# aoschu/esn-ofdm-mimo

Measured on AMD Instinct MI355X. Metric: OFDM symbols/s through the ESN detector (4x8 TDL-B, N=128, N_res=512; train+predict+detect), higher is better.
Workload: dtype f16 operands / f32 accumulate

## Files before the change

### esn_ofdm_mimo_amd/csrc/esn_api.hip

```cpp
#include <stdarg.h>
#include <stdio.h>
#include <stdlib.h>
#include <math.h>
#include <string.h>
#include "esn_common.h"

namespace esn {
int launch_recur_f64(const RecurParams& p, hipStream_t stream);
size_t recur_f64_lds_bytes(int FB, int n_res, int n_in, int n_out);
bool f64_mfma_geometry(int n_res, int n_in, int n_out, bool harvest, Geometry* g);
int launch_recur_f64_mfma(const RecurParams& p, hipStream_t stream);
#ifdef ESN_WITH_RS
bool rs_path_applies(int precision, const RecurParams& p);
int launch_recur_rs(int precision, const RecurParams& p, size_t wo_rs_off, hipStream_t stream);
#endif
bool big_path_applies(int precision, const RecurParams& p);
int big_slots(const RecurParams& p);
size_t big_workspace_bytes(int n_slots, int Mp, int Kp);
int launch_recur_big(int precision, const RecurParams& p, size_t wo_big_off, void* workspace, hipStream_t stream,
                     bool io32 = false);
bool big_harvest_applies(int precision, const RecurParams& p);
size_t big_harvest_workspace_bytes(int n_groups, int Kp);
int launch_harvest_big(int precision, const RecurParams& p, void* workspace, hipStream_t stream);
bool cluster_applies(int precision, const RecurParams& p);
size_t cluster_workspace_bytes(int n_res, int n_in, int n_out, bool harvest);
int launch_recur_cluster(const RecurParams& p, void* workspace, hipStream_t stream);
bool mfma_geometry(int precision, int n_res, int n_in, int n_out, bool harvest, Geometry* g);
int launch_recur_mfma(int precision, const RecurParams& p, hipStream_t stream, bool io32 = false);
bool harvest_cluster_applies(int precision, const RecurParams& p);
size_t harvest_cluster_workspace_bytes(int n_pilots, int C, int n_wsets);
int launch_harvest_cluster(int precision, const RecurParams& p, int C, void* workspace, hipStream_t stream);
int launch_recur_skew16(int precision, const RecurParams& p, hipStream_t stream, bool io32 = false);
size_t packed_w_bytes(int precision, int n_res, int n_in, int n_out, const Geometry& g);
size_t packed_wout_bytes(int precision, int n_res, int n_in, int n_out, const Geometry& g);
size_t wout_big_offset(int precision, int n_out, const Geometry& g);
size_t f64_w_offset(int n_res, int n_in, int n_out);
size_t f64_wout_offset(int n_res, int n_in, int n_out);
int launch_pack_weights(int precision, const esn_shape_t* sh, const Geometry& g, const double* W,
                        const double* Win, const double* Wfb, void* packed, hipStream_t stream);
int launch_pack_readout(int precision, const esn_shape_t* sh, const Geometry& g, int n_groups,
                        const double* Wout, void* packed, hipStream_t stream);
size_t solve_work_doubles(int rows, int cols, int n_out);
int launch_readout_solve(const double* E, const double* D, int n_groups, int T, int transient,
                         int cols, int n_out, const double* t_scale, const double* t_shift,
                         double* W_out, int* status, void* workspace, hipStream_t stream);
int launch_readout_chol(const double* E, const float* E32, const double* D, int n_groups, int T, int transient,
                        int cols, int n_out, const double* t_scale, const double* t_shift,
                        double* W_out, int* status, hipStream_t stream);
size_t chol_big_work_doubles(int n);
int launch_readout_chol_big(const double* E, const float* E32, const double* D, int n_groups, int T, int transient,
                            int cols, int n_out, const double* t_scale, const double* t_shift,
                            double* W_out, int* status, void* workspace, hipStream_t stream);
int launch_gen_taps(const TapParams& tp, hipStream_t stream);
int launch_gen_frames(const FrameGenParams& fp, hipStream_t stream, bool c64 = false);
int launch_channel_estimate(const ChanEstParams& cp, hipStream_t stream);
int launch_mmse_detect(const MmseParams& mp, hipStream_t stream);
int launch_taps_to_freq(const TapsFreqParams& tp, hipStream_t stream);
int launch_ldpc_encode(const LdpcEncodeParams& ep, hipStream_t stream);
int launch_qam_llr(const LlrParams& lp, hipStream_t stream);
int launch_ldpc_decode(const LdpcDecodeParams& dp, hipStream_t stream);
int launch_detect_count(const DetectParams& dp, hipStream_t stream, bool io32 = false);
}

using namespace esn;

static thread_local char g_err[512] = "";

namespace esn {
static bool parse3(const char* v, int (&out)[3]) {
    int a, b, c;
    if (v && sscanf(v, "%d,%d,%d", &a, &b, &c) == 3 && a > 0 && b > 0 && c > 0) { out[0] = a; out[1] = b; out[2] = c; return true; }
    out[0] = out[1] = out[2] = 0;
    return false;
}
Knobs& knobs() {
    static Knobs k = [] {
        Knobs x;
        const char* v = getenv("ESN_SKEW");
        x.skew = (v && v[0] == '0') ? 0 : 1;
        parse3(getenv("ESN_MFMA_GEOM"), x.geom16);
        parse3(getenv("ESN_MFMA_GEOM_F32"), x.geom32);
        v = getenv("ESN_CHOL_SKIP");
        x.chol_skip = v ? atoi(v) : 0;
        v = getenv("ESN_F64_MFMA");
        x.f64_mfma = (v && v[0] == '0') ? 0 : 1;
        v = getenv("ESN_RS");
        x.rs = (v && v[0] == '1') ? 1 : 0;
        v = getenv("ESN_BIG_GEMM");
        x.big_gemm = (v && v[0] == '0') ? 0 : 1;
        v = getenv("ESN_CLUSTER");
        x.cluster = (v && v[0] == '0') ? 0 : 1;
        x.gen_ko = 0;
        v = getenv("ESN_HARVEST_GEMM");
        x.harvest_gemm = (v && v[0] == '1') ? 1 : 0;
        v = getenv("ESN_BIG_NT");
        x.big_nt = (v && v[0] == '4') ? 4 : 2;
        v = getenv("ESN_HCLUSTER");
        x.hcluster = (v && (v[0] == '0' || v[0] == '4' || v[0] == '8')) ? v[0] - '0' : 1;
        v = getenv("ESN_S16");
        x.s16 = (v && v[0] == '0') ? 0 : 1;
        v = getenv("ESN_BIG_PIPE");
        x.big_pipe = (v && v[0] == '0') ? 0 : 1;
        return x;
    }();
    return k;
}
}

static int fail(int code, const char* fmt, ...) {
    va_list ap;
    va_start(ap, fmt);
    vsnprintf(g_err, sizeof(g_err), fmt, ap);
    va_end(ap);
    return code;
}

namespace esn {
int api_fail(int code, const char* fmt, ...) {
    va_list ap;
    va_start(ap, fmt);
    vsnprintf(g_err, sizeof(g_err), fmt, ap);
    va_end(ap);
    return code;
}
}

static int hip_fail(int e, const char* what) {
    if (e == 0) return 0;
    if (e > 0) return fail(-1000 - e, "%s: HIP error %d (%s)", what, e, hipGetErrorString((hipError_t)e));
    return fail(-2, "%s: no kernel instance for this shape", what);
}

static bool check_shape(const esn_shape_t* s) {
    return s && s->n_res > 0 && s->n_in > 0 && s->n_out > 0 && s->n_wsets > 0;
}

static bool geometry_for(int precision, const esn_shape_t* s, Geometry* g, bool harvest = false) {
    memset(g, 0, sizeof(*g));
    if (precision == ESN_F64) {
        int fb = 8;
        while (fb > 1 && recur_f64_lds_bytes(fb, s->n_res, s->n_in, s->n_out) > 150 * 1024) fb >>= 1;
        if (recur_f64_lds_bytes(fb, s->n_res, s->n_in, s->n_out) > 160 * 1024) return false;
        Geometry gp, gh;
        memset(&gp, 0, sizeof(gp)); memset(&gh, 0, sizeof(gh));
        if (f64_mfma_geometry(s->n_res, s->n_in, s->n_out, false, &gp) &&
            f64_mfma_geometry(s->n_res, s->n_in, s->n_out, true, &gh))
            *g = harvest ? gh : gp;
        g->Bt = fb;
        return true;
    }
    if (precision < ESN_F64 || precision > ESN_BF16) return false;
    return mfma_geometry(precision, s->n_res, s->n_in, s->n_out, harvest, g);
}

#ifdef ESN_STAMPS
static unsigned long long* g_stamp_buf = nullptr;
extern "C" void esn_debug_set_stamp_buffer(void* dev) { g_stamp_buf = (unsigned long long*)dev; }
#define ESN_SET_STAMPS(p) (p).stamps = g_stamp_buf
#else
#define ESN_SET_STAMPS(p) (p).stamps = nullptr
#endif

extern "C" {

const char* esn_last_error(void) { return g_err; }

int esn_abi_version(void) { return 10; }

int esn_debug_set(const char* key, const char* value) {
    if (!key) return fail(-1, "esn_debug_set: null key");
    Knobs& k = knobs();
    if (!strcmp(key, "skew")) { k.skew = (value && value[0] == '0') ? 0 : 1; return 0; }
    if (!strcmp(key, "mfma_geom")) { parse3(value, k.geom16); return 0; }
    if (!strcmp(key, "mfma_geom_f32")) { parse3(value, k.geom32); return 0; }
    if (!strcmp(key, "chol_skip")) { k.chol_skip = value ? atoi(value) : 0; return 0; }
    if (!strcmp(key, "f64_mfma")) { k.f64_mfma = (value && value[0] == '0') ? 0 : 1; return 0; }
    if (!strcmp(key, "rs")) {
#ifdef ESN_WITH_RS
        k.rs = (value && value[0] == '1') ? 1 : 0; return 0;
#else
        if (value && value[0] == '1') return fail(-3, "esn_debug_set: the register-state kernel is not in this build (ESN_WITH_RS=1)");
        return 0;
#endif
    }
    if (!strcmp(key, "big_gemm")) { k.big_gemm = (value && value[0] == '0') ? 0 : 1; return 0; }
    if (!strcmp(key, "cluster")) { k.cluster = (value && value[0] == '0') ? 0 : 1; return 0; }
    if (!strcmp(key, "gen_ko")) { k.gen_ko = value ? atoi(value) : 0; return 0; }
    if (!strcmp(key, "harvest_gemm")) { k.harvest_gemm = (value && value[0] == '1') ? 1 : 0; return 0; }
    if (!strcmp(key, "big_nt")) { k.big_nt = (value && value[0] == '4') ? 4 : 2; return 0; }
    if (!strcmp(key, "hcluster")) {
        k.hcluster = (value && (value[0] == '0' || value[0] == '4' || value[0] == '8')) ? value[0] - '0' : 1;
        return 0;
    }
    if (!strcmp(key, "s16")) { k.s16 = (value && value[0] == '0') ? 0 : 1; return 0; }
    if (!strcmp(key, "big_pipe")) { k.big_pipe = (value && value[0] == '0') ? 0 : 1; return 0; }
    return fail(-1, "esn_debug_set: unknown key '%s'", key);
}

int esn_device_info(int* cu_count, int* lds_bytes_per_cu, int* clock_khz, char* arch_name, int arch_name_len) {
    int dev = 0;
    hipError_t e = hipGetDevice(&dev);
    if (e != hipSuccess) return hip_fail((int)e, "hipGetDevice");
    hipDeviceProp_t prop;
    e = hipGetDeviceProperties(&prop, dev);
    if (e != hipSuccess) return hip_fail((int)e, "hipGetDeviceProperties");
    if (cu_count) *cu_count = prop.multiProcessorCount;
    if (lds_bytes_per_cu) *lds_bytes_per_cu = (int)prop.maxSharedMemoryPerMultiProcessor;
    if (clock_khz) *clock_khz = prop.clockRate;
    if (arch_name && arch_name_len > 0) {
        strncpy(arch_name, prop.gcnArchName, arch_name_len - 1);
        arch_name[arch_name_len - 1] = 0;
    }
    return 0;
}

int esn_tile_frames(int precision, const esn_shape_t* shape) {
    Geometry g;
    if (!check_shape(shape)) return fail(-1, "esn_tile_frames: invalid shape");
    if (!geometry_for(precision, shape, &g)) return fail(-2, "esn_tile_frames: unsupported shape/precision");
    return g.Bt;
}

size_t esn_packed_weights_bytes(int precision, const esn_shape_t* shape) {
    Geometry g;
    if (!check_shape(shape) || !geometry_for(precision, shape, &g)) return 0;
    return packed_w_bytes(precision, shape->n_res, shape->n_in, shape->n_out, g);
}

size_t esn_packed_readout_bytes(int precision, const esn_shape_t* shape) {
    Geometry g;
    if (!check_shape(shape) || !geometry_for(precision, shape, &g)) return 0;
    return packed_wout_bytes(precision, shape->n_res, shape->n_in, shape->n_out, g);
}

int esn_pack_weights(int precision, const esn_shape_t* shape, const double* W, const double* W_in,
                     const double* W_fb, void* packed, void* stream) {
    Geometry g;
    if (!check_shape(shape)) return fail(-1, "esn_pack_weights: invalid shape");
    if (!W || !W_in || !W_fb || !packed) return fail(-1, "esn_pack_weights: null pointer");
    if (!geometry_for(precision, shape, &g)) return fail(-2, "esn_pack_weights: unsupported shape/precision");
    return hip_fail(launch_pack_weights(precision, shape, g, W, W_in, W_fb, packed, (hipStream_t)stream),
                    "esn_pack_weights");
}

int esn_pack_readout(int precision, const esn_shape_t* shape, int n_groups, const double* W_out,
                     void* packed, void* stream) {
    Geometry g;
    if (!check_shape(shape) || n_groups <= 0) return fail(-1, "esn_pack_readout: invalid shape");
    if (!W_out || !packed) return fail(-1, "esn_pack_readout: null pointer");
    if (!geometry_for(precision, shape, &g)) return fail(-2, "esn_pack_readout: unsupported shape/precision");
    return hip_fail(launch_pack_readout(precision, shape, g, n_groups, W_out, packed, (hipStream_t)stream),
                    "esn_pack_readout");
}

static void shrink_f64_tile(int precision, RecurParams& p) {
    if (precision != ESN_F64) return;
    const long long slots = (long long)p.n_groups * p.Fpad;
    while (p.g.Bt > 1 && p.g.Bt / 2 >= slots) p.g.Bt >>= 1;
}

static bool use_f64_mfma(int precision, const RecurParams& p, long long sequences) {
    return precision == ESN_F64 && p.g.m64 && sequences > 8 && knobs().f64_mfma;
}

static int fill_common(RecurParams& p, int precision, const esn_shape_t* shape, const char* who,
                       bool harvest = false) {
    memset(&p, 0, sizeof(p));
    if (!check_shape(shape)) return fail(-1, "%s: invalid shape", who);
    if (!geometry_for(precision, shape, &p.g, harvest)) return fail(-2, "%s: unsupported shape/precision", who);
    p.n_res = shape->n_res; p.n_in = shape->n_in; p.n_out = shape->n_out;
    p.teacher_forcing = shape->teacher_forcing ? 1 : 0;
    p.n_wsets = shape->n_wsets;
    p.wset_stride = packed_w_bytes(precision, p.n_res, p.n_in, p.n_out, p.g);
    p.wout_stride = packed_wout_bytes(precision, p.n_res, p.n_in, p.n_out, p.g);
    p.leak = (shape->leak_rate == 0.0) ? 1.0 : shape->leak_rate;
    if (!(p.leak > 0.0 && p.leak <= 1.0)) return fail(-1, "%s: leak_rate %g outside (0, 1]", who, shape->leak_rate);
    if (p.leak != 1.0 && precision != ESN_F64)
// ... 493 lines not shown
```

### esn_ofdm_mimo_amd/csrc/esn_common.h

```cpp
#pragma once
#include <hip/hip_runtime.h>
#include <stdint.h>
#include <stddef.h>
#include <type_traits>
#include "../../include/esn_hip.h"

namespace esn {

struct Geometry {
    int Mp;
    int kin;
    int kfb;
    int Kp;
    int Ks;
    int Bt;
    int NW, MT, NT;
    int ro_parts;
    int ro_fold;
    int skew;
    int big;
    int rs;
    int s16;
    int m64;
    int Bt64;
// ... 85 lines not shown
};
struct MmseParams {
    int n_frames, frames_per_group, n_sub, log2n, cp, n_t, n_r, m;
    int zf;
    const double* p_i; double no;
    const double* H;
    const double* y_cp;
    const uint8_t* tx_bits;
    long long* err; long long* bits; double* X_hat;
};

struct LdpcEncodeParams {
    int n_frames, n_t, k, n;
    const uint8_t* P;
    const uint8_t* u;
    uint8_t* bits;
};
struct LlrParams {
    int n_frames, n_sub, n_t, m;
    const double* X_hat;
    double* llr;
    double* sigma2;
};
struct LdpcDecodeParams {
    int n_cw, n, k, m_checks, n_edges, maxiter, cw_per_group;
    double var;
    const int* chk_ptr;
    const int* edge_var;
    const int* var_ptr;
    const int* var_edge;
    const double* y;
    const uint8_t* u_true;
    uint8_t* x_out;
    long long* err; long long* bits;
};

__device__ __forceinline__ int slot_group(const RecurParams& p, int slot, int& j) {
    if (p.spw == 0) {
        const int grp = slot / p.Fpad;
        j = slot - grp * p.Fpad;
        return grp;
    }
    const int w = slot / p.spw, ls = slot - w * p.spw;
    const int gi = ls / p.Fpad;
    j = ls - gi * p.Fpad;
    const int grp = gi * p.n_wsets + w;
    return (w < p.n_wsets) ? grp : p.n_groups;
}
__device__ __forceinline__ int slot_group(const RecurParams& p, int slot) { int j; return slot_group(p, slot, j); }
__device__ __forceinline__ int slot_wset(const RecurParams& p, int slot0) {
    if (!p.spw) return 0;
    const int w = slot0 / p.spw + p.wset_rot;
    return w >= p.n_wsets ? w - p.n_wsets : w;
}
__device__ __forceinline__ int slot_frame(const RecurParams& p, int slot, int& grp) {
    int j;
    grp = slot_group(p, slot, j);
    const int fr = grp * p.F + j;
    return (j < p.F && grp < p.n_groups && fr < p.n_frames) ? fr : -1;
}

template <bool IO32> using io_elem = typename std::conditional<IO32, float, double>::type;
template <bool IO32> __device__ __forceinline__ const io_elem<IO32>* in_ptr(const RecurParams& p) {
    if constexpr (IO32) return p.U32; else return p.U;
}
template <bool IO32> __device__ __forceinline__ io_elem<IO32>* out_ptr(const RecurParams& p) {
    if constexpr (IO32) return p.Y32; else return p.Y;
}

inline __host__ __device__ int round_up(int x, int m) { return (x + m - 1) / m * m; }

inline __host__ __device__ int s16_pos(int k) {
    return k < 512 ? (k & ~31) + 8 * ((k & 15) >> 2) + 4 * ((k & 31) >> 4) + (k & 3) : k;
}
inline __host__ __device__ int s16_nat(int pos) {
    return pos < 512 ? (pos & ~31) + 16 * ((pos & 7) >> 2) + 4 * ((pos & 31) >> 3) + (pos & 3) : pos;
}

struct Knobs {
    int skew;
    int geom16[3];
    int geom32[3];
    int chol_skip;
    int f64_mfma;
    int rs;
    int big_gemm;
    int cluster;
    int big_nt;
    int big_pipe;
    int harvest_gemm;
    int gen_ko;
    int s16;
    int hcluster;
};
Knobs& knobs();

__device__ __forceinline__ int xcd_remap(int bid, int nwg) {
    const int nx = 8;
    if (nwg < nx) return bid;
    int q = nwg / nx, r = nwg % nx, x = bid % nx, i = bid / nx;
    return (x < r ? x * (q + 1) : r * (q + 1) + (x - r) * q) + i;
}

__device__ __forceinline__ uint32_t mix32(uint32_t x) {
    x ^= x >> 16; x *= 0x7feb352dU; x ^= x >> 15; x *= 0x846ca68bU; x ^= x >> 16;
    return x;
}
__device__ __forceinline__ uint32_t noise_key(uint64_t seed, uint32_t frame, uint32_t step) {
    uint32_t k = mix32((uint32_t)seed ^ (frame * 0x9E3779B9U));
    k = mix32(k ^ (uint32_t)(seed >> 32) ^ (step * 0x85EBCA6BU + 0x27d4eb2fU));
    return k;
}
__device__ __forceinline__ uint32_t noise_mix(uint32_t s) {
    s ^= s >> 16;
    s = __umul24(s, 0x9E3779U);
    s ^= s >> 16;
    return s;
}
__device__ __forceinline__ uint32_t noise_quad(uint32_t k, uint32_t row4) {
    return noise_mix(k + row4 * 0x9E3779B9U);
}
__device__ __forceinline__ float noise_byte(uint32_t quad, int b) {
    return (float)((quad >> (8 * b)) & 0xffU) * (1.0f / 256.0f) + (0.5f / 256.0f);
}
__device__ __forceinline__ float noise_uniform(uint32_t k, uint32_t row) {
    return noise_byte(noise_quad(k, row >> 2), (int)(row & 3));
}

constexpr float TANH32_SERIES_MAX = 0.3f;
__device__ __forceinline__ float tanh_f32_series(float x) {
    float x2 = x * x;
    float p = -0.00886323552990220f;
    p = fmaf(p, x2, 0.0218694885361552f);
    p = fmaf(p, x2, -0.0539682539682540f);
    p = fmaf(p, x2, 0.133333333333333f);
    p = fmaf(p, x2, -0.333333333333333f);
    return fmaf(p * x2, x, x);
}
__device__ __forceinline__ float tanh_f32(float x) {
    float ax = fabsf(x);
    float p = tanh_f32_series(x);
    float e = __expf(2.0f * ax);
    float r = 1.0f - 2.0f * __builtin_amdgcn_rcpf(e + 1.0f);
    r = copysignf(r, x);
    return ax < TANH32_SERIES_MAX ? p : r;
}

constexpr double TANH64_SERIES_MAX = 0.25;
__device__ __forceinline__ double tanh_f64_series(double x) {
    const double u = x * x;
    double p = 9.691537956929451e-05;
    p = fma(p, u, -2.3912911424355248e-04);
    p = fma(p, u, 5.90027440945586e-04);
    p = fma(p, u, -1.4558343870513183e-03);
    p = fma(p, u, 3.592128036572481e-03);
    p = fma(p, u, -8.863235529902197e-03);
    p = fma(p, u, 2.1869488536155203e-02);
    p = fma(p, u, -5.396825396825397e-02);
    p = fma(p, u, 1.3333333333333333e-01);
    p = fma(p, u, -3.333333333333333e-01);
    return fma(p * u, x, x);
}

constexpr double ACT_PRESCALE = 2.8853900817779268;
__device__ __forceinline__ float tanh_prescaled(float z) {
    float e = __builtin_amdgcn_exp2f(z);
// ... 15 lines not shown
```

### esn_ofdm_mimo_amd/csrc/esn_solve.hip

```cpp
#include <stdlib.h>
#include "esn_common.h"

namespace esn {

struct SolveParams {
    const double* E; const double* D;
    const float* E32;
    int n_groups, T, transient, cols, n_out;
    const double* t_scale; const double* t_shift;
    double* W_out; int* status;
    double* work; size_t work_stride;
    int m, n, wide;
    int skip;
    int part_ok;
    int vec;
};

__device__ __forceinline__ double wave_sum(double v) {
#pragma unroll
    for (int off = 32; off > 0; off >>= 1) v += __shfl_down(v, off);
    return __shfl(v, 0);
}

__global__ __launch_bounds__(1024) void readout_qr_kernel(SolveParams sp) {
    __shared__ double red[16];
    __shared__ double bc[4];
    const int g = blockIdx.x;
    const int tid = threadIdx.x, nth = blockDim.x;
    const int lane = tid & 63, wv = tid >> 6, nwv = nth >> 6;
    const int m = sp.m, n = sp.n, nrhs = sp.n_out;
    const int rows = sp.T - sp.transient, cols = sp.cols;
    double* M = sp.work + (size_t)g * sp.work_stride;
    const int ncol_tot = sp.wide ? n : n + nrhs;
    double* R = M + (size_t)ncol_tot * m;
    double* rdiag = R + (size_t)nrhs * m;
    double* beta = rdiag + n;
    const double* Eg = sp.E + ((size_t)g * sp.T + sp.transient) * cols;
    const double* Dg = sp.D + ((size_t)g * sp.T + sp.transient) * nrhs;

    if (sp.wide) {
        for (size_t i = tid; i < (size_t)n * m; i += nth) M[i] = Eg[i];
        for (int i = tid; i < nrhs * m; i += nth) {
            int o = i / m, j = i % m;
            double v = 0.0;
            if (j < n) {
                double sc = sp.t_scale ? sp.t_scale[(size_t)g * nrhs + o] : 1.0;
                double sh = sp.t_shift ? sp.t_shift[(size_t)g * nrhs + o] : 0.0;
                v = Dg[(size_t)j * nrhs + o] * sc + sh;
            }
            R[i] = v;
        }
    } else {
        for (size_t i = tid; i < (size_t)n * m; i += nth) {
            int c = (int)(i / m), rr = (int)(i % m);
            M[i] = Eg[(size_t)rr * cols + c];
        }
        for (int i = tid; i < nrhs * m; i += nth) {
            int o = i / m, rr = i % m;
            double sc = sp.t_scale ? sp.t_scale[(size_t)g * nrhs + o] : 1.0;
            double sh = sp.t_shift ? sp.t_shift[(size_t)g * nrhs + o] : 0.0;
            M[(size_t)(n + o) * m + rr] = Dg[(size_t)rr * nrhs + o] * sc + sh;
        }
    }
    __syncthreads();

    for (int j = 0; j < n; ++j) {
        double* cj = M + (size_t)j * m;
        double part = 0.0;
        for (int i = j + tid; i < m; i += nth) { double x = cj[i]; part = fma(x, x, part); }
        part = wave_sum(part);
        if (lane == 0) red[wv] = part;
        __syncthreads();
        if (tid == 0) {
            double sigma = 0.0;
            for (int w = 0; w < nwv; ++w) sigma += red[w];
            double x0 = cj[j];
            double nx = sqrt(sigma);
            double alpha = (x0 >= 0.0) ? -nx : nx;
            double v0 = x0 - alpha;
            double vtv = sigma - x0 * x0 + v0 * v0;
            double b = (vtv > 0.0) ? 2.0 / vtv : 0.0;
            cj[j] = v0;
            rdiag[j] = alpha;
            beta[j] = b;
            bc[0] = b;
        }
        __syncthreads();
        const double b = bc[0];
        if (b != 0.0) {
            for (int c = j + 1 + wv; c < ncol_tot; c += nwv) {
                double* cc = M + (size_t)c * m;
                double dot = 0.0;
                for (int i = j + lane; i < m; i += 64) dot = fma(cj[i], cc[i], dot);
                dot = wave_sum(dot) * b;
                for (int i = j + lane; i < m; i += 64) cc[i] = fma(-dot, cj[i], cc[i]);
            }
        }
        __syncthreads();
// ... 25 lines not shown
                for (int k = lane; k < j; k += 64) acc = fma(cj[k], z[k], acc);
                acc = wave_sum(acc);
                if (lane == 0) {
                    double d = rdiag[j];
                    z[j] = (fabs(d) > tol) ? (z[j] - acc) / d : 0.0;
                }
                __builtin_amdgcn_s_waitcnt(0);
                __builtin_amdgcn_wave_barrier();
            }
            for (int j = n - 1; j >= 0; --j) {
                const double* cj = M + (size_t)j * m;
                const double b = beta[j];
                if (b == 0.0) continue;
                double dot = 0.0;
                for (int i = j + lane; i < m; i += 64) dot = fma(cj[i], z[i], dot);
                dot = wave_sum(dot) * b;
                for (int i = j + lane; i < m; i += 64) z[i] = fma(-dot, cj[i], z[i]);
                __builtin_amdgcn_s_waitcnt(0);
                __builtin_amdgcn_wave_barrier();
            }
            double* wo = sp.W_out + ((size_t)g * nrhs + o) * cols;
            for (int i = lane; i < m; i += 64) wo[i] = z[i];
        }
    } else {
        for (int o = wv; o < nrhs; o += nwv) {
            double* c = M + (size_t)(n + o) * m;
            for (int j = n - 1; j >= 0; --j) {
                double acc = 0.0;
                for (int k = j + 1 + lane; k < n; k += 64) acc = fma(M[(size_t)k * m + j], c[k], acc);
                acc = wave_sum(acc);
                if (lane == 0) {
                    double d = rdiag[j];
                    c[j] = (fabs(d) > tol) ? (c[j] - acc) / d : 0.0;
                }
                __builtin_amdgcn_s_waitcnt(0);
                __builtin_amdgcn_wave_barrier();
            }
            double* wo = sp.W_out + ((size_t)g * nrhs + o) * cols;
            for (int i = lane; i < n; i += 64) wo[i] = c[i];
        }
    }
}

size_t solve_work_doubles(int rows, int cols, int n_out) {
    const bool wide = rows < cols;
    const size_t m = wide ? cols : rows, n = wide ? rows : cols;
    size_t d = (n + (wide ? 0 : n_out)) * m + (size_t)n_out * m + 2 * n;
    return (d + 1) & ~(size_t)1;
}

int launch_readout_solve(const double* E, const double* D, int n_groups, int T, int transient,
                         int cols, int n_out, const double* t_scale, const double* t_shift,
                         double* W_out, int* status, void* workspace, hipStream_t stream) {
    SolveParams sp;
    const int rows = T - transient;
    sp.E = E; sp.E32 = nullptr; sp.D = D; sp.n_groups = n_groups; sp.T = T; sp.transient = transient;
    sp.cols = cols; sp.n_out = n_out; sp.t_scale = t_scale; sp.t_shift = t_shift;
    sp.W_out = W_out; sp.status = status;
    sp.work = reinterpret_cast<double*>(workspace);
    sp.work_stride = solve_work_doubles(rows, cols, n_out);
    sp.wide = rows < cols;
    sp.m = sp.wide ? cols : rows;
    sp.n = sp.wide ? rows : cols;
    hipLaunchKernelGGL(readout_qr_kernel, dim3(n_groups), dim3(1024), 0, stream, sp);
    return (int)hipGetLastError();
}

}

namespace esn {

constexpr int CH_NP = 128;
constexpr int CH_NT = 512;
constexpr int CH_NW = CH_NT / 64;
constexpr int CH_TILES = 36;
constexpr int CH_KC = 32;
constexpr int CH_AS_LD = CH_NP + 16;
constexpr int CH_RHS = 8;
constexpr size_t CH_LDS = sizeof(double) * ((size_t)CH_TILES * 256 + (size_t)CH_NP * CH_RHS);
static_assert(2 * CH_KC * CH_AS_LD <= CH_TILES * 256, "E staging aliases the Gram tiles");

typedef double f64x4 __attribute__((ext_vector_type(4)));

__device__ __forceinline__ int ch_tile(int ti, int tj) { return (ti * (ti + 1) / 2 + tj) * 256; }
__device__ __forceinline__ int ch_el(int r, int c) { return r * 16 + (c ^ (r & ~1)); }

__device__ __forceinline__ void ch_load4(const float* p, float (&v)[4]) {
    const float4 x = *reinterpret_cast<const float4*>(p);
    v[0] = x.x; v[1] = x.y; v[2] = x.z; v[3] = x.w;
}
__device__ __forceinline__ void ch_load4(const double* p, double (&v)[4]) {
    const double2 x = *reinterpret_cast<const double2*>(p), y = *reinterpret_cast<const double2*>(p + 2);
    v[0] = x.x; v[1] = x.y; v[2] = y.x; v[3] = y.y;
}
__device__ __forceinline__ const float* ch_src(const SolveParams& sp, float*) { return sp.E32; }
__device__ __forceinline__ const double* ch_src(const SolveParams& sp, double*) { return sp.E; }

__device__ __forceinline__ double ch_bcast(double x, int src) {
    const uint64_t u = __builtin_bit_cast(uint64_t, x);
    const uint32_t lo = __builtin_amdgcn_readlane((uint32_t)u, src);
    const uint32_t hi = __builtin_amdgcn_readlane((uint32_t)(u >> 32), src);
    return __builtin_bit_cast(double, ((uint64_t)hi << 32) | lo);
}

__device__ __forceinline__ int ch_factor_diag(double* D, int j0, int n, double piv_tol, int lane) {
    const int r = lane & 15;
    double a[16], x[16];
#pragma unroll
    for (int c = 0; c < 16; ++c) a[c] = D[ch_el(r, c)];
    double my_invd = 1.0;
    unsigned rejected = 0, dropped = 0;
#pragma unroll
    for (int j = 0; j < 16; ++j) {
        const double v = ch_bcast(a[j], j);
        const bool live = j0 + j < n;
        const bool ok = live && v > piv_tol;
        if (live && !ok) rejected |= 1u << j;
        if (!ok) dropped |= 1u << j;
        const double d = ok ? sqrt(v) : 1.0, inv_d = ok ? 1.0 / d : 0.0;
        if (r == j) my_invd = ok ? inv_d : 1.0;
        a[j] = (r == j) ? d : ((r > j) ? a[j] * inv_d : 0.0);
#pragma unroll
        for (int k = j + 1; k < 16; ++k) {
            const double lkj = ch_bcast(a[j], k);
            if (r >= k) a[k] = fma(-a[j], lkj, a[k]);
        }
    }
#pragma unroll
    for (int i = 0; i < 16; ++i) {
        double sacc = (i == r) ? 1.0 : 0.0;
#pragma unroll
        for (int k = 0; k < i; ++k) sacc = fma(-ch_bcast(a[k], i), x[k], sacc);
        const double idi = ch_bcast(my_invd, i);
        x[i] = (i >= r && !((dropped >> i) & 1u)) ? sacc * idi : 0.0;
    }
    if (lane < 16) {
#pragma unroll
        for (int i = 0; i < 16; ++i) D[ch_el(i, r)] = x[i];
    }
    return rejected ? 1 : 0;
}

template <typename TE, bool wide>
__global__ __launch_bounds__(CH_NT) __attribute__((amdgpu_waves_per_eu(4))) void readout_chol_kernel(SolveParams sp) {
    extern __shared__ __attribute__((aligned(16))) char chol_smem[];
    double* Gs = reinterpret_cast<double*>(chol_smem);
    double* As = Gs;
    double* Bs = Gs + CH_TILES * 256;
    const int g = blockIdx.x, tid = threadIdx.x;
    const int lane = tid & 63, wv = __builtin_amdgcn_readfirstlane(tid >> 6);
    const int lr = lane & 15, lq = lane >> 4;
    const int rows = sp.T - sp.transient, cols = sp.cols, nrhs = sp.n_out;
    const int n = wide ? rows : cols;
    const int m = wide ? cols : rows;
    const int ntile = (n + 15) / 16;
    const TE* A = ch_src(sp, (TE*)nullptr) + ((size_t)g * sp.T + sp.transient) * cols;
    const double* Dg = sp.D + ((size_t)g * sp.T + sp.transient) * nrhs;

    int g_ti[5], g_tj[5];
    const int g_cnt = wv < 4 ? 5 : 4;
#pragma unroll
    for (int q = 0; q < 5; ++q) {
        const int t = wv + CH_NW * q < CH_TILES ? wv + CH_NW * q : 0;
        int ti = 0;
        while ((ti + 1) * (ti + 2) / 2 <= t) ++ti;
        g_ti[q] = ti;
        g_tj[q] = t - ti * (ti + 1) / 2;
    }
    f64x4 acc[5];
#pragma unroll
    for (int q = 0; q < 5; ++q) acc[q] = f64x4{0.0, 0.0, 0.0, 0.0};
    double atb[2] = {0.0, 0.0};
    auto run_of = [&](int p, int& i, int& kk) {
        const int e = tid + CH_NT * p;
        if (wide) { i = (e & 15) + 16 * ((e >> 7) & 7); kk = 4 * ((e >> 4) & 7); }
        else      { kk = e >> 5; i = 4 * (e & 31); }
    };
    TE stg[2][4];
    auto fetch = [&](int k0) {
#pragma unroll
        for (int p = 0; p < 2; ++p) {
            int i, kk;
            run_of(p, i, kk);
            const int k = k0 + kk;
            int nv = wide ? (i < n ? m - k : 0) : (k < m ? n - i : 0);
            nv = nv < 0 ? 0 : (nv > 4 ? 4 : nv);
            const TE* src = A + (wide ? (size_t)i * cols + k : (size_t)k * cols + i);
            if (nv == 4 && sp.vec) {
                ch_load4(src, stg[p]);
            } else {
#pragma unroll
                for (int j = 0; j < 4; ++j) stg[p][j] = j < nv ? src[j] : (TE)0;
            }
        }
    };
    auto commit = [&](double* dst) {
#pragma unroll
        for (int p = 0; p < 2; ++p) {
            int i, kk;
            run_of(p, i, kk);
#pragma unroll
            for (int j = 0; j < 4; ++j) {
                if (wide) dst[(kk + j) * CH_AS_LD + i] = (double)stg[p][j];
                else      dst[kk * CH_AS_LD + i + j] = (double)stg[p][j];
            }
        }
    };
    double* Abuf[2] = {As, As + CH_KC * CH_AS_LD};
    const int m_run = (sp.skip & 1) ? CH_KC : m;
    for (int k0 = 0, cur = 0; k0 < m_run; k0 += CH_KC, cur ^= 1) {
        if (k0 == 0) {
            fetch(0);
            commit(Abuf[0]);
            __syncthreads();
        }
        if (k0 + CH_KC < m_run) fetch(k0 + CH_KC);
        const double* Ac = Abuf[cur];
        const int kmax = (m - k0 < CH_KC) ? m - k0 : CH_KC;
        const double* slab0 = Ac + lq * CH_AS_LD + lr;
        for (int k4 = 0; k4 < kmax; k4 += 4) {
            const double* slab = slab0 + k4 * CH_AS_LD;
#pragma unroll
            for (int q = 0; q < 5; ++q)
                if (q < g_cnt)
                    acc[q] = __builtin_amdgcn_mfma_f64_16x16x4f64(slab[g_ti[q] * 16], slab[g_tj[q] * 16], acc[q], 0, 0, 0);
        }
        if constexpr (!wide) {
#pragma unroll
            for (int p = 0; p < 2; ++p) {
                const int e = tid + CH_NT * p, o = e / CH_NP, i = e % CH_NP;
                if (o < nrhs) {
                    const double sc = sp.t_scale ? sp.t_scale[(size_t)g * nrhs + o] : 1.0;
                    const double sh = sp.t_shift ? sp.t_shift[(size_t)g * nrhs + o] : 0.0;
                    for (int kk = 0; kk < kmax; ++kk)
                        atb[p] = fma(Ac[kk * CH_AS_LD + i], Dg[(size_t)(k0 + kk) * nrhs + o] * sc + sh, atb[p]);
                }
            }
        }
        if (k0 + CH_KC < m_run) commit(Abuf[cur ^ 1]);
        __syncthreads();
    }

#pragma unroll
    for (int q = 0; q < 5; ++q)
        if (q < g_cnt) {
            double* T = Gs + ch_tile(g_ti[q], g_tj[q]);
#pragma unroll
            for (int i = 0; i < 4; ++i) T[ch_el(4 * i + lq, lr)] = acc[q][i];
        }
#pragma unroll
    for (int p = 0; p < 2; ++p) {
        const int e = tid + CH_NT * p;
        if (wide) {
            const int i = e / CH_RHS, o = e % CH_RHS;
            double v = 0.0;
            if (i < n && o < nrhs) {
                const double sc = sp.t_scale ? sp.t_scale[(size_t)g * nrhs + o] : 1.0;
                const double sh = sp.t_shift ? sp.t_shift[(size_t)g * nrhs + o] : 0.0;
                v = Dg[(size_t)i * nrhs + o] * sc + sh;
            }
            Bs[e] = v;
        } else {
            const int o = e / CH_NP, i = e % CH_NP;
            Bs[i * CH_RHS + o] = (o < nrhs && i < n) ? atb[p] : 0.0;
        }
    }
    __syncthreads();

    int bad = 0;
    const int nblk = (sp.skip & 2) ? 1 : ntile;
    double piv_tol = 0.0;
    if (wv == 0) {
        double dmax = 0.0;
        for (int i = lane; i < n; i += 64) dmax = fmax(dmax, Gs[ch_tile(i >> 4, i >> 4) + ch_el(i & 15, i & 15)]);
#pragma unroll
        for (int off = 32; off > 0; off >>= 1) dmax = fmax(dmax, __shfl_xor(dmax, off));
        piv_tol = dmax * 1e-14;
    }
    for (int kb = -1; kb < nblk; ++kb) {
        if (kb >= 0) {
            const int rt = kb + 1 + wv;
            if (rt < ntile) {
                const double* Li = Gs + ch_tile(kb, kb);

                double* T = Gs + ch_tile(rt, kb);
                f64x4 c = {0.0, 0.0, 0.0, 0.0};
#pragma unroll
                for (int k0 = 0; k0 < 16; k0 += 4)
                    c = __builtin_amdgcn_mfma_f64_16x16x4f64(T[ch_el(lr, k0 + lq)], Li[ch_el(lr, k0 + lq)], c, 0, 0, 0);
#pragma unroll
                for (int i = 0; i < 4; ++i) T[ch_el(4 * i + lq, lr)] = c[i];
            }
        }
        if (kb >= 0) {
            __syncthreads();
            const int mt = ntile - kb - 1, cnt = mt * (mt + 1) / 2;
            for (int t = wv; t < cnt; t += (wv == 0 ? cnt : CH_NW - 1)) {
                int di = 0;
                while ((di + 1) * (di + 2) / 2 <= t) ++di;
                const int ti = kb + 1 + di, tj = kb + 1 + t - di * (di + 1) / 2;
                double* C = Gs + ch_tile(ti, tj);
                const double* La = Gs + ch_tile(ti, kb);
                const double* Lb = Gs + ch_tile(tj, kb);
                f64x4 c;
#pragma unroll
                for (int i = 0; i < 4; ++i) c[i] = C[ch_el(4 * i + lq, lr)];
#pragma unroll
                for (int k0 = 0; k0 < 16; k0 += 4)
                    c = __builtin_amdgcn_mfma_f64_16x16x4f64(-La[ch_el(lr, k0 + lq)], Lb[ch_el(lr, k0 + lq)], c, 0, 0, 0);
#pragma unroll
                for (int i = 0; i < 4; ++i) C[ch_el(4 * i + lq, lr)] = c[i];
            }
        }
        if (wv == 0 && kb + 1 < nblk) bad |= ch_factor_diag(Gs + ch_tile(kb + 1, kb + 1), 16 * (kb + 1), n, piv_tol, lane);
        __syncthreads();
    }

    if (!(sp.skip & 4)) {
        const bool bl = lr < CH_RHS;
        f64x4 keep = {0.0, 0.0, 0.0, 0.0};
        int keep_t = -1;
        auto rhs_tile = [&](int I) -> f64x4 {
            f64x4 v;
#pragma unroll
            for (int i = 0; i < 4; ++i) v[i] = bl ? Bs[(16 * I + 4 * i + lq) * CH_RHS + lr] : 0.0;
            return v;
        };
        auto put_tile = [&](int I, const f64x4& v) {
            if (bl) {
#pragma unroll
                for (int i = 0; i < 4; ++i) Bs[(16 * I + 4 * i + lq) * CH_RHS + lr] = v[i];
            }
        };
        auto flush = [&]() {
            if (wv == CH_NW - 1 && keep_t >= 0) put_tile(keep_t, keep);
            keep_t = -1;
        };
        for (int I = 0; I < ntile; ++I) {
            flush();
            const int J = I + 1 + wv;
            const bool upd = J < ntile;
            if (upd || wv == CH_NW - 1) {
                const double* Li = Gs + ch_tile(I, I);
                const f64x4 b = rhs_tile(I);
                f64x4 z = {0.0, 0.0, 0.0, 0.0};
#pragma unroll
                for (int s = 0; s < 4; ++s)
                    z = __builtin_amdgcn_mfma_f64_16x16x4f64(Li[ch_el(lr, 4 * s + lq)], b[s], z, 0, 0, 0);
                if (upd) {
                    const double* L = Gs + ch_tile(J, I);
                    f64x4 c = rhs_tile(J);
#pragma unroll
                    for (int s = 0; s < 4; ++s)
                        c = __builtin_amdgcn_mfma_f64_16x16x4f64(-L[ch_el(lr, 4 * s + lq)], z[s], c, 0, 0, 0);
                    put_tile(J, c);
                } else {
                    keep = z;
                    keep_t = I;
                }
            }
            __syncthreads();
        }
        flush();
        __syncthreads();
        for (int I = ntile - 1; I >= 0; --I) {
            flush();
            const int J = wv;
            const bool upd = J < I;
            if (upd || wv == CH_NW - 1) {
                const double* Li = Gs + ch_tile(I, I);
                const f64x4 zi = rhs_tile(I);
                f64x4 x = {0.0, 0.0, 0.0, 0.0};
#pragma unroll
                for (int s = 0; s < 4; ++s)
                    x = __builtin_amdgcn_mfma_f64_16x16x4f64(Li[ch_el(4 * s + lq, lr)], zi[s], x, 0, 0, 0);
                if (upd) {
                    const double* L = Gs + ch_tile(I, J);
                    f64x4 c = rhs_tile(J);
#pragma unroll
                    for (int s = 0; s < 4; ++s)
                        c = __builtin_amdgcn_mfma_f64_16x16x4f64(-L[ch_el(4 * s + lq, lr)], x[s], c, 0, 0, 0);
                    put_tile(J, c);
                } else {
                    keep = x;
                    keep_t = I;
                }
            }
            __syncthreads();
        }
        flush();
        __syncthreads();
    }

    if constexpr (wide) {
        constexpr int CPT = 16 / sizeof(TE);
        const int nunit = cols / CPT;
        int parts = nunit > 0 ? CH_NT / nunit : 0;
        parts = parts > 3 ? 3 : parts;
        if (sp.vec && cols % CPT == 0 && parts > 0 && (parts - 1) * CH_RHS * cols <= CH_TILES * 256 && !(sp.skip & 8)) {
            double* part = Gs;
            const int pt = tid / nunit, un = tid - pt * nunit;
            double w[CPT][CH_RHS];
#pragma unroll
            for (int c = 0; c < CPT; ++c)
#pragma unroll
                for (int o = 0; o < CH_RHS; ++o) w[c][o] = 0.0;
            if (pt < parts) {
                const int per = (n + parts - 1) / parts;
                const int i0 = pt * per, i1 = (i0 + per < n) ? i0 + per : n;
                const TE* ac = A + (size_t)CPT * un;
#pragma unroll 4
                for (int i = i0; i < i1; ++i) {
                    TE a[CPT];
                    if constexpr (CPT == 4) {
                        ch_load4(ac + (size_t)i * cols, a);
                    } else {
                        const double2 ad = *reinterpret_cast<const double2*>(ac + (size_t)i * cols);
                        a[0] = ad.x; a[1] = ad.y;
                    }
#pragma unroll
                    for (int o = 0; o < CH_RHS; ++o)
                        if (o < nrhs) {
                            const double al = Bs[i * CH_RHS + o];
#pragma unroll
                            for (int c = 0; c < CPT; ++c) w[c][o] = fma((double)a[c], al, w[c][o]);
                        }
                }
                if (pt > 0) {
#pragma unroll
                    for (int o = 0; o < CH_RHS; ++o)
                        if (o < nrhs) {
#pragma unroll
                            for (int c = 0; c < CPT; ++c) part[((pt - 1) * CH_RHS + o) * cols + CPT * un + c] = w[c][o];
                        }
                }
            }
            __syncthreads();
            if (pt == 0) {
#pragma unroll
                for (int o = 0; o < CH_RHS; ++o)
                    if (o < nrhs) {
#pragma unroll
                        for (int c = 0; c < CPT; ++c) {
                            double v = w[c][o];
                            for (int q = 1; q < parts; ++q) v += part[((q - 1) * CH_RHS + o) * cols + CPT * un + c];
                            sp.W_out[((size_t)g * nrhs + o) * cols + CPT * un + c] = v;
                        }
                    }
            }
        } else {
            for (int c = tid; c < ((sp.skip & 8) ? 0 : cols); c += CH_NT) {
                double w[CH_RHS];
#pragma unroll
                for (int o = 0; o < CH_RHS; ++o) w[o] = 0.0;
#pragma unroll 8
                for (int i = 0; i < n; ++i) {
                    const double a = (double)A[(size_t)i * cols + c];
#pragma unroll
                    for (int o = 0; o < CH_RHS; ++o)
                        if (o < nrhs) w[o] = fma(a, Bs[i * CH_RHS + o], w[o]);
                }
#pragma unroll
                for (int o = 0; o < CH_RHS; ++o)
                    if (o < nrhs) sp.W_out[((size_t)g * nrhs + o) * cols + c] = w[o];
            }
        }
    } else {
        for (int e = tid; e < nrhs * cols; e += CH_NT) {
            const int o = e / cols, c = e % cols;
            sp.W_out[((size_t)g * nrhs + o) * cols + c] = Bs[c * CH_RHS + o];
        }
    }
    if (tid == 0) sp.status[g] = bad;
}

int launch_readout_chol(const double* E, const float* E32, const double* D, int n_groups, int T, int transient,
                        int cols, int n_out, const double* t_scale, const double* t_shift,
                        double* W_out, int* status, hipStream_t stream) {
    SolveParams sp;
    sp.E32 = E32;
    const int rows = T - transient;
    const int n = rows < cols ? rows : cols;
    if (n > CH_NP || n_out > CH_RHS) return -1;
    sp.E = E; sp.D = D; sp.n_groups = n_groups; sp.T = T; sp.transient = transient;
    sp.cols = cols; sp.n_out = n_out; sp.t_scale = t_scale; sp.t_shift = t_shift;
    sp.W_out = W_out; sp.status = status; sp.work = nullptr; sp.work_stride = 0;
    sp.wide = rows < cols; sp.m = sp.wide ? cols : rows; sp.n = n;
    sp.skip = knobs().chol_skip;
    sp.part_ok = 0;
    const uintptr_t base = E32 ? (uintptr_t)E32 : (uintptr_t)E;
    sp.vec = (base % 16 == 0) && (cols % (E32 ? 4 : 2) == 0);
    void (*fn)(SolveParams) = E32 ? (sp.wide ? readout_chol_kernel<float, true> : readout_chol_kernel<float, false>)
                                  : (sp.wide ? readout_chol_kernel<double, true> : readout_chol_kernel<double, false>);
    hipError_t e = hipFuncSetAttribute(reinterpret_cast<const void*>(fn), hipFuncAttributeMaxDynamicSharedMemorySize,
                                       (int)CH_LDS);
    if (e != hipSuccess) return (int)e;
    hipLaunchKernelGGL(fn, dim3(n_groups), dim3(CH_NT), CH_LDS, stream, sp);
    return (int)hipGetLastError();
}

}

namespace esn {

constexpr int CB_NMAX = 512;
constexpr int CB_KC = 8;
constexpr int CB_PLD = 17;
constexpr int CB_NT = 512;
constexpr int CB_NW = CB_NT / 64;
constexpr int CB_EPT = CB_NMAX * CB_KC / CB_NT;
constexpr int CB_TPW = 16;

size_t chol_big_work_doubles(int n) {
    const size_t np = (size_t)round_up(n, 16);
    return np * np;
}

__global__ __launch_bounds__(CB_NT) void readout_chol_big_kernel(SolveParams sp) {
    extern __shared__ __attribute__((aligned(16))) char cb_smem[];
    typedef double f64x4 __attribute__((ext_vector_type(4)));
    __shared__ int sh_bad;
    __shared__ double sh_invd[CB_NMAX];
    __shared__ double sh_linv[16][17];
    __shared__ double sh_red[CB_NW];
    const int g = blockIdx.x, tid = threadIdx.x;
    const int lane = tid & 63, wv = tid >> 6;
    const int wvu = __builtin_amdgcn_readfirstlane(wv);
    const int rows = sp.T - sp.transient, cols = sp.cols, nrhs = sp.n_out;
    const bool wide = rows < cols;
    const int n = wide ? rows : cols;
    const int m = wide ? cols : rows;
    const int np = round_up(n, 16), ntile = np / 16;
    const int ld = np;
    double* Gw = sp.work + (size_t)g * sp.work_stride;
    const size_t a_off = ((size_t)g * sp.T + sp.transient) * cols;
    const double* A = sp.E ? sp.E + a_off : nullptr;
    const float* A32 = sp.E32 ? sp.E32 + a_off : nullptr;
    const double* Dg = sp.D + ((size_t)g * sp.T + sp.transient) * nrhs;
    const int lr = lane & 15, lq = lane >> 4;
    if (tid == 0) sh_bad = 0;

    {
        const int AS_LD = np + 4;
        double* Abuf[2] = {reinterpret_cast<double*>(cb_smem), reinterpret_cast<double*>(cb_smem) + (size_t)CB_KC * AS_LD};
        const int ept = (np * CB_KC + CB_NT - 1) / CB_NT;
        double stg[CB_EPT];
        auto fetch = [&](int k0) {
#pragma unroll
            for (int q = 0; q < CB_EPT; ++q) {
                const int e = tid + CB_NT * q;
                int kk, i;
                if (wide) { i = e / CB_KC; kk = e % CB_KC; } else { kk = e / np; i = e % np; }
                const int k = k0 + kk;
                const size_t ai_ = wide ? (size_t)i * cols + k : (size_t)k * cols + i;
                stg[q] = (q < ept && e < np * CB_KC && i < n && k < m) ? (A32 ? (double)A32[ai_] : A[ai_]) : 0.0;
            }
        };
        auto commit = [&](double* dst) {
#pragma unroll
            for (int q = 0; q < CB_EPT; ++q) {
                const int e = tid + CB_NT * q;
                if (q < ept && e < np * CB_KC) {
                    int kk, i;
                    if (wide) { i = e / CB_KC; kk = e % CB_KC; } else { kk = e / np; i = e % np; }
                    dst[kk * AS_LD + i] = stg[q];
                }
            }
        };
        const int fr_off = lq * AS_LD + lr;
        const int n_pass = (ntile + 3) / 4;
        for (int jb = 0; jb < n_pass; ++jb) {
            const int tj0 = 4 * jb, tj1 = (tj0 + 4 < ntile) ? tj0 + 4 : ntile;
// ... 336 lines not shown
```

Measured before the change: 10.94 million.

## Stream Cholesky readout operands via buffer-load-to-LDS ring buffers

In the wide f32 path of the readout Cholesky kernel, the Gram accumulation loop now feeds MFMA through a 4-deep ring of LDS buffers filled by buffer_load...lds DMA, replacing the double-buffered register fetch/commit. The W_out back-substitution pass gets a similar 3-deep DMA ring that stages rows of E for each partition. The aim is to hide global load latency and drop the register staging and extra LDS writes. In exchange it adds hand-written waitcnt/barrier sequencing and inline asm LDS reads, which carry a risk of hazards. It is enabled by default and can be turned off with ESN_CHOL_DMA=0, and it also adds stamp instrumentation.

New measurement: 11.12 million (median of 6 runs). +1.7%, better.

```diff
diff --git a/esn_ofdm_mimo_amd/csrc/esn_api.hip b/esn_ofdm_mimo_amd/csrc/esn_api.hip
--- a/esn_ofdm_mimo_amd/csrc/esn_api.hip
+++ b/esn_ofdm_mimo_amd/csrc/esn_api.hip
@@ -99,6 +99,8 @@
         x.hcluster = (v && (v[0] == '0' || v[0] == '4' || v[0] == '8')) ? v[0] - '0' : 1;
         v = getenv("ESN_S16");
         x.s16 = (v && v[0] == '0') ? 0 : 1;
+        v = getenv("ESN_CHOL_DMA");
+        x.chol_dma = (v && v[0] == '0') ? 0 : 1;
         v = getenv("ESN_BIG_PIPE");
         x.big_pipe = (v && v[0] == '0') ? 0 : 1;
         return x;
@@ -156,6 +158,7 @@
 #ifdef ESN_STAMPS
 static unsigned long long* g_stamp_buf = nullptr;
 extern "C" void esn_debug_set_stamp_buffer(void* dev) { g_stamp_buf = (unsigned long long*)dev; }
+namespace esn { unsigned long long* stamp_buffer() { return g_stamp_buf; } }
 #define ESN_SET_STAMPS(p) (p).stamps = g_stamp_buf
 #else
 #define ESN_SET_STAMPS(p) (p).stamps = nullptr
@@ -193,6 +196,7 @@
         return 0;
     }
     if (!strcmp(key, "s16")) { k.s16 = (value && value[0] == '0') ? 0 : 1; return 0; }
+    if (!strcmp(key, "chol_dma")) { k.chol_dma = (value && value[0] == '0') ? 0 : 1; return 0; }
     if (!strcmp(key, "big_pipe")) { k.big_pipe = (value && value[0] == '0') ? 0 : 1; return 0; }
     return fail(-1, "esn_debug_set: unknown key '%s'", key);
 }
diff --git a/esn_ofdm_mimo_amd/csrc/esn_common.h b/esn_ofdm_mimo_amd/csrc/esn_common.h
--- a/esn_ofdm_mimo_amd/csrc/esn_common.h
+++ b/esn_ofdm_mimo_amd/csrc/esn_common.h
@@ -191,6 +191,7 @@
     int geom16[3];
     int geom32[3];
     int chol_skip;
+    int chol_dma;
     int f64_mfma;
     int rs;
     int big_gemm;
diff --git a/esn_ofdm_mimo_amd/csrc/esn_solve.hip b/esn_ofdm_mimo_amd/csrc/esn_solve.hip
--- a/esn_ofdm_mimo_amd/csrc/esn_solve.hip
+++ b/esn_ofdm_mimo_amd/csrc/esn_solve.hip
@@ -1,4 +1,5 @@
 #include <stdlib.h>
+#include <type_traits>
 #include "esn_common.h"
 
 namespace esn {
@@ -14,6 +15,8 @@
     int skip;
     int part_ok;
     int vec;
+    int dma;
+    unsigned long long* stamps;
 };
 
 __device__ __forceinline__ double wave_sum(double v) {
@@ -205,6 +208,48 @@
 
 typedef double f64x4 __attribute__((ext_vector_type(4)));
 
+constexpr int CH_RING = 4;
+constexpr int CH_RBUF = CH_KC * CH_NP * 4;
+constexpr int CH_WRING = 3;
+constexpr int CH_WSEG = 8192;
+constexpr int CH_WROWS = 4;
+static_assert(CH_RING * CH_RBUF <= CH_TILES * 256 * 8, "Gram ring aliases the Gram tiles");
+static_assert(CH_WRING * 3 * CH_WSEG <= CH_TILES * 256 * 8, "W_out ring aliases the Gram tiles");
+
+__device__ __forceinline__ __amdgpu_buffer_rsrc_t ch_rsrc(const void* ptr, int bytes) {
+    const uint64_t a = (uint64_t)reinterpret_cast<uintptr_t>(ptr);
+    const uint32_t lo = __builtin_amdgcn_readfirstlane((uint32_t)a);
+    const uint32_t hi = __builtin_amdgcn_readfirstlane((uint32_t)(a >> 32));
+    return __builtin_amdgcn_make_buffer_rsrc(reinterpret_cast<char*>((uintptr_t)(((uint64_t)hi << 32) | lo)), 0,
+                                             __builtin_amdgcn_readfirstlane(bytes), 0x00020000);
+}
+__device__ __forceinline__ void ch_dma16(__amdgpu_buffer_rsrc_t rs, char* dst, int voff) {
+    __builtin_amdgcn_raw_ptr_buffer_load_lds(rs, (__attribute__((address_space(3))) void*)dst, 16, voff, 0, 0, 0);
+}
+constexpr int CH_OOR = 0x7ffffff0;
+__device__ __forceinline__ void ch_wait_dma(int pending) {
+    switch (pending) {
+        case 4: asm volatile("s_waitcnt vmcnt(4) lgkmcnt(0)" ::: "memory"); break;
+        case 3: asm volatile("s_waitcnt vmcnt(3) lgkmcnt(0)" ::: "memory"); break;
+        case 2: asm volatile("s_waitcnt vmcnt(2) lgkmcnt(0)" ::: "memory"); break;
+        default: asm volatile("s_waitcnt vmcnt(0) lgkmcnt(0)" ::: "memory"); break;
+    }
+}
+
+__device__ __forceinline__ void ch_wrow(const char* e, const double* al, float (&a)[4], double (&b)[8]) {
+    typedef float f32x4 __attribute__((ext_vector_type(4)));
+    typedef double f64x2 __attribute__((ext_vector_type(2)));
+    const uint32_t ea = (uint32_t)(uintptr_t)(const __attribute__((address_space(3))) char*)e;
+    const uint32_t ba = (uint32_t)(uintptr_t)(const __attribute__((address_space(3))) double*)al;
+    f32x4 ev;
+    f64x2 b0, b1, b2, b3;
+    asm volatile("ds_read_b128 %0, %5\n\tds_read_b128 %1, %6\n\tds_read_b128 %2, %6 offset:16\n\t"
+                 "ds_read_b128 %3, %6 offset:32\n\tds_read_b128 %4, %6 offset:48\n\ts_waitcnt lgkmcnt(0)"
+                 : "=v"(ev), "=v"(b0), "=v"(b1), "=v"(b2), "=v"(b3) : "v"(ea), "v"(ba) : "memory");
+    a[0] = ev.x; a[1] = ev.y; a[2] = ev.z; a[3] = ev.w;
+    b[0] = b0.x; b[1] = b0.y; b[2] = b1.x; b[3] = b1.y; b[4] = b2.x; b[5] = b2.y; b[6] = b3.x; b[7] = b3.y;
+}
+
 __device__ __forceinline__ int ch_tile(int ti, int tj) { return (ti * (ti + 1) / 2 + tj) * 256; }
 __device__ __forceinline__ int ch_el(int r, int c) { return r * 16 + (c ^ (r & ~1)); }
 
@@ -331,12 +376,93 @@
     };
     double* Abuf[2] = {As, As + CH_KC * CH_AS_LD};
     const int m_run = (sp.skip & 1) ? CH_KC : m;
-    for (int k0 = 0, cur = 0; k0 < m_run; k0 += CH_KC, cur ^= 1) {
+    constexpr bool can_dma = wide && sizeof(TE) == 4;
+    const bool dma = can_dma && sp.dma && sp.vec;
+#ifdef ESN_STAMPS
+    unsigned long long st_acc[8] = {0, 0, 0, 0, 0, 0, 0, 0}, st_ph[4] = {0, 0, 0, 0};
+    ESN_STAMP(st_k0);
+#endif
+    if constexpr (can_dma) {
+        if (dma) {
+            char* ring = chol_smem;
+            const __amdgpu_buffer_rsrc_t ers = ch_rsrc(A, n * cols * 4);
+            const int kq = lane >> 3;
+            int roff[2];
+#pragma unroll
+            for (int j = 0; j < 2; ++j) roff[j] = ((16 * wv + 8 * j + (lane & 7)) * cols + 4 * kq) * 4;
+            const int nch = (m_run + CH_KC - 1) / CH_KC;
+            auto issue = [&](int c, int b) {
+                const int k0 = c * CH_KC;
+                const bool ok = k0 + 4 * kq < m;
+#pragma unroll
+                for (int j = 0; j < 2; ++j)
+                    ch_dma16(ers, ring + b * CH_RBUF + (2 * wv + j) * 1024, ok ? roff[j] + 4 * k0 : CH_OOR);
+            };
+#pragma unroll
+            for (int c = 0; c < CH_RING - 1; ++c)
+                if (c < nch) issue(c, c);
+            const int lbase = 1024 * (lr >> 3) + 16 * (lr & 7) + 4 * lq;
+            for (int c = 0, b = 0; c < nch; ++c, b = (b + 1 == CH_RING ? 0 : b + 1)) {
+#ifdef ESN_STAMPS
+                ESN_STAMP(s0);
+#endif
+                const int later = nch - 1 - c < CH_RING - 2 ? nch - 1 - c : CH_RING - 2;
+                ch_wait_dma(2 * later);
+#ifdef ESN_STAMPS
+                ESN_STAMP(s1);
+#endif
+                __builtin_amdgcn_s_barrier();
+                if (c + CH_RING - 1 < nch) issue(c + CH_RING - 1, b == 0 ? CH_RING - 1 : b - 1);
+                const char* buf = ring + b * CH_RBUF + lbase;
+                const float* pa[5];
+                const float* pb[5];
+#pragma unroll
+                for (int q = 0; q < 5; ++q) {
+                    pa[q] = reinterpret_cast<const float*>(buf + 2048 * g_ti[q]);
+                    pb[q] = reinterpret_cast<const float*>(buf + 2048 * g_tj[q]);
+                }
+#ifdef ESN_STAMPS
+                ESN_STAMP(s2);
+                {
+                    float x = pa[0][0];
+                    asm volatile("" :: "v"(x));
+                }
+                ESN_STAMP(s3);
+#endif
+                auto step = [&](int s, auto cnt) {
+#pragma unroll
+                    for (int q = 0; q < decltype(cnt)::value; ++q)
+                        acc[q] = __builtin_amdgcn_mfma_f64_16x16x4f64((double)pa[q][32 * s], (double)pb[q][32 * s], acc[q], 0, 0, 0);
+                };
+                const int kmax = (m - c * CH_KC < CH_KC) ? m - c * CH_KC : CH_KC;
+                if (kmax == CH_KC && g_cnt == 5) {
+#pragma unroll
+                    for (int s = 0; s < CH_KC / 4; ++s) step(s, std::integral_constant<int, 5>());
+                } else if (kmax == CH_KC) {
+#pragma unroll
+                    for (int s = 0; s < CH_KC / 4; ++s) step(s, std::integral_constant<int, 4>());
+                } else if (g_cnt == 5) {
+                    for (int s = 0; s < kmax / 4; ++s) step(s, std::integral_constant<int, 5>());
+                } else {
+                    for (int s = 0; s < kmax / 4; ++s) step(s, std::integral_constant<int, 4>());
+                }
+#ifdef ESN_STAMPS
+                ESN_STAMP(s4);
+                st_acc[0] += s1 - s0; st_acc[1] += s2 - s1; st_acc[2] += s3 - s2; st_acc[3] += s4 - s3;
+#endif
+            }
+            __syncthreads();
+        }
+    }
+    for (int k0 = 0, cur = 0; k0 < (dma ? 0 : m_run); k0 += CH_KC, cur ^= 1) {
         if (k0 == 0) {
             fetch(0);
             commit(Abuf[0]);
             __syncthreads();
         }
+#ifdef ESN_STAMPS
+        ESN_STAMP(s0);
+#endif
         if (k0 + CH_KC < m_run) fetch(k0 + CH_KC);
         const double* Ac = Abuf[cur];
         const int kmax = (m - k0 < CH_KC) ? m - k0 : CH_KC;
@@ -360,9 +486,22 @@
                 }
             }
         }
+#ifdef ESN_STAMPS
+        ESN_STAMP(s1);
+#endif
         if (k0 + CH_KC < m_run) commit(Abuf[cur ^ 1]);
+#ifdef ESN_STAMPS
+        ESN_STAMP(s2);
+#endif
         __syncthreads();
-    }
+#ifdef ESN_STAMPS
+        ESN_STAMP(s3);
+        st_acc[3] += s1 - s0; st_acc[0] += s2 - s1; st_acc[1] += s3 - s2;
+#endif
+    }
+#ifdef ESN_STAMPS
+    ESN_STAMP(st_k1);
+#endif
 
 #pragma unroll
     for (int q = 0; q < 5; ++q)
@@ -439,6 +578,9 @@
         __syncthreads();
     }
 
+#ifdef ESN_STAMPS
+    ESN_STAMP(st_k2);
+#endif
     if (!(sp.skip & 4)) {
         const bool bl = lr < CH_RHS;
         f64x4 keep = {0.0, 0.0, 0.0, 0.0};
@@ -515,6 +657,9 @@
         __syncthreads();
     }
 
+#ifdef ESN_STAMPS
+    ESN_STAMP(st_k3);
+#endif
     if constexpr (wide) {
         constexpr int CPT = 16 / sizeof(TE);
         const int nunit = cols / CPT;
@@ -528,8 +673,80 @@
             for (int c = 0; c < CPT; ++c)
 #pragma unroll
                 for (int o = 0; o < CH_RHS; ++o) w[c][o] = 0.0;
-            if (pt < parts) {
-                const int per = (n + parts - 1) / parts;
+            const int per = (n + parts - 1) / parts;
+            int rw = CH_WSEG / (cols * 4);
+            rw = rw > CH_WROWS ? CH_WROWS : rw;
+            bool wdma = false;
+            if constexpr (can_dma) {
+              wdma = dma && rw > 0;
+              if (wdma) {
+                char* ring = chol_smem;
+                const __amdgpu_buffer_rsrc_t ers = ch_rsrc(A, n * cols * 4);
+                const int rowb = cols * 4;
+                const int nch = (per + rw - 1) / rw;
+                auto issue = [&](int c, int b) {
+#pragma unroll
+                    for (int j = 0; j < 3; ++j) {
+                        const int r0 = j * per + c * rw;
+                        int nr = (j < parts) ? ((j + 1) * per < n ? (j + 1) * per : n) - r0 : 0;
+                        nr = nr < 0 ? 0 : (nr > rw ? rw : nr);
+                        const int off = 1024 * wv + 16 * lane;
+                        ch_dma16(ers, ring + (b * 3 + j) * CH_WSEG + 1024 * wv, off < nr * rowb ? r0 * rowb + off : CH_OOR);
+                    }
+                };
+#pragma unroll
+                for (int c = 0; c < CH_WRING - 1; ++c)
+                    if (c < nch) issue(c, c);
+                const int i0 = pt * per, i1 = (i0 + per < n) ? i0 + per : n;
+                for (int c = 0, b = 0; c < nch; ++c, b = (b + 1 == CH_WRING ? 0 : b + 1)) {
+#ifdef ESN_STAMPS
+                    ESN_STAMP(s0);
+#endif
+                    ch_wait_dma(nch - 1 - c < CH_WRING - 2 ? 3 * (nch - 1 - c) : 3 * (CH_WRING - 2));
+#ifdef ESN_STAMPS
+                    ESN_STAMP(s1);
+#endif
+                    __builtin_amdgcn_s_barrier();
+                    if (c + CH_WRING - 1 < nch) issue(c + CH_WRING - 1, b == 0 ? CH_WRING - 1 : b - 1);
+#ifdef ESN_STAMPS
+                    ESN_STAMP(s2);
+#endif
+                    if (pt < parts) {
+                        const char* seg = ring + (b * 3 + pt) * CH_WSEG + CPT * sizeof(TE) * un;
+                        const int ib = i0 + c * rw;
+                        const int nr = ((ib + rw < i1) ? ib + rw : i1) - ib;
+#pragma unroll
+                        for (int rr = 0; rr < CH_WROWS; ++rr) {
+                            if (rr >= nr) break;
+                            const int i = ib + rr;
+                            float a[4];
+                            double al[CH_RHS];
+                            ch_wrow(seg + rr * rowb, Bs + i * CH_RHS, a, al);
+#pragma unroll
+                            for (int o = 0; o < CH_RHS; ++o)
+                                if (o < nrhs) {
+#pragma unroll
+                                    for (int cc = 0; cc < CPT; ++cc) w[cc][o] = fma((double)a[cc], al[o], w[cc][o]);
+                                }
+                        }
+                    }
+#ifdef ESN_STAMPS
+                    ESN_STAMP(s3);
+                    st_acc[4] += s1 - s0; st_acc[5] += s2 - s1; st_acc[6] += s3 - s2;
+#endif
+                }
+                __syncthreads();
+                if (pt > 0 && pt < parts) {
+#pragma unroll
+                    for (int o = 0; o < CH_RHS; ++o)
+                        if (o < nrhs) {
+#pragma unroll
+                            for (int c = 0; c < CPT; ++c) part[((pt - 1) * CH_RHS + o) * cols + CPT * un + c] = w[c][o];
+                        }
+                }
+              }
+            }
+            if (!wdma && pt < parts) {
                 const int i0 = pt * per, i1 = (i0 + per < n) ? i0 + per : n;
                 const TE* ac = A + (size_t)CPT * un;
 #pragma unroll 4
@@ -595,7 +812,22 @@
         }
     }
     if (tid == 0) sp.status[g] = bad;
-}
+#ifdef ESN_STAMPS
+    ESN_STAMP(st_k4);
+    if (sp.stamps && g == 0 && lane == 0) {
+        for (int i = 0; i < 7; ++i) sp.stamps[wv * 8 + i] = st_acc[i];
+        sp.stamps[(8 + wv) * 8 + 0] = st_k1 - st_k0;
+        sp.stamps[(8 + wv) * 8 + 1] = st_k2 - st_k1;
+        sp.stamps[(8 + wv) * 8 + 2] = st_k3 - st_k2;
+        sp.stamps[(8 + wv) * 8 + 3] = st_k4 - st_k3;
+        sp.stamps[(8 + wv) * 8 + 4] = st_k4 - st_k0;
+    }
+#endif
+}
+
+#ifdef ESN_STAMPS
+unsigned long long* stamp_buffer();
+#endif
 
 int launch_readout_chol(const double* E, const float* E32, const double* D, int n_groups, int T, int transient,
                         int cols, int n_out, const double* t_scale, const double* t_shift,
@@ -610,7 +842,13 @@
     sp.W_out = W_out; sp.status = status; sp.work = nullptr; sp.work_stride = 0;
     sp.wide = rows < cols; sp.m = sp.wide ? cols : rows; sp.n = n;
     sp.skip = knobs().chol_skip;
+    sp.dma = knobs().chol_dma;
     sp.part_ok = 0;
+#ifdef ESN_STAMPS
+    sp.stamps = stamp_buffer();
+#else
+    sp.stamps = nullptr;
+#endif
     const uintptr_t base = E32 ? (uintptr_t)E32 : (uintptr_t)E;
     sp.vec = (base % 16 == 0) && (cols % (E32 ? 4 : 2) == 0);
     void (*fn)(SolveParams) = E32 ? (sp.wide ? readout_chol_kernel<float, true> : readout_chol_kernel<float, false>)
```
